# matteospanio/torchfx

Hardware: AMD Instinct MI355X
Metric: Msamples/s/GPU (64-ch fused biquad→FIR→FFT-conv chain); % HBM roofline (higher is better)
Workload: dtype f64 (IIR) + f32 (FFT); f32 I/O

## Files before the change

### torchfx_amd/csrc/ols_kernels.h

```cpp
#pragma once
#include "common.h"
#include "epilogue.h"
#include "fftpk.h"

namespace tfx {

typedef float2 cpx;

__device__ __forceinline__ cpx cmul(cpx a, cpx b) { return make_float2(a.x * b.x - a.y * b.y, a.x * b.y + a.y * b.x); }
__device__ __forceinline__ cpx cmulc(cpx a, cpx b) { return make_float2(a.x * b.x + a.y * b.y, a.y * b.x - a.x * b.y); }
__device__ __forceinline__ cpx cadd(cpx a, cpx b) { return make_float2(a.x + b.x, a.y + b.y); }
__device__ __forceinline__ cpx csub(cpx a, cpx b) { return make_float2(a.x - b.x, a.y - b.y); }

template <bool INV>
__device__ __forceinline__ void dft4(cpx &a0, cpx &a1, cpx &a2, cpx &a3)
{
    const cpx s02 = cadd(a0, a2), d02 = csub(a0, a2), s13 = cadd(a1, a3), d13 = csub(a1, a3);
    const cpx id = INV ? make_float2(-d13.y, d13.x) : make_float2(d13.y, -d13.x);
    a0 = cadd(s02, s13);
    a2 = csub(s02, s13);
    a1 = cadd(d02, id);
    a3 = csub(d02, id);
}

__device__ __forceinline__ void wave_sync2()
{
    __builtin_amdgcn_fence(__ATOMIC_RELEASE, "wavefront");
    __builtin_amdgcn_wave_barrier();
    __builtin_amdgcn_fence(__ATOMIC_ACQUIRE, "wavefront");
}

struct OlsGeom {
    int64_t Tn;
    int64_t Tout;
    int64_t F;
    int64_t S;
    int64_t t0;
    int64_t pad_left;
    int64_t out_shift;
    int64_t nframes;
    const float *hist;
    int64_t H;
    float ep_gain;
    int ep_scale, ep_clamp, ep_stat;
    double *ep_partial;
    int64_t ep_row;
    int N2;
    int P2;
    int sh_on, sh_base;
    int *nf_flag;
    int *nf_pair;
    int nt;
};

constexpr int OLS_N1 = 256;
constexpr int OLS_CB = 32;

__device__ __forceinline__ int pad16(int p) { return p + (p >> 4); }
__device__ __forceinline__ int row_shift(const OlsGeom &g, int64_t c) { return g.sh_on ? (int)(((int64_t)g.sh_base + c * g.Tn) & 31) : 0; }


template <bool INV, int NBF, bool LEAN = false>
__device__ __forceinline__ void col_stages16(cpx (&v)[NBF][16], cpx *lds, const cpx *tw256, int col, int q)
{
    constexpr int QS = 16 / NBF;
    using pk::v2f;
    const v2f Wc = {0.92387953251128675613f, 0.38268343236508977173f}, Wr = {0.70710678118654752440f, 0.70710678118654752440f};
    v2f *L = (v2f *)lds;
    const v2f *TW = (const v2f *)tw256;
#pragma unroll
    for (int i = 0; i < NBF; ++i) {
        v2f u[16];
#pragma unroll
        for (int t = 0; t < 16; ++t) u[t] = __builtin_bit_cast(v2f, v[i][t]);
        pk::pk_dft16<INV>(u, Wc, Wr);
        const int j = q + QS * i;
#pragma unroll
        for (int k = 0; k < 16; ++k) L[(16 * j + k) * OLS_CB + col] = u[PK_DFT16_AT(k)];
    }
    __syncthreads();
#pragma unroll
    for (int i = 0; i < NBF; ++i) {
        const int j = q + QS * i;
        v2f d[16], w[16];
#pragma unroll
        for (int t = 0; t < 16; ++t) d[t] = L[(j + 16 * t) * OLS_CB + col];
        if (LEAN) {
#pragma unroll
            for (int b = 0; b < 4; ++b) {
#pragma unroll
                for (int t = 0; t < 4; ++t) if (4 * b + t > 0) w[t] = TW[((4 * b + t) * j) & 255];
                __builtin_amdgcn_sched_barrier(0);
#pragma unroll
                for (int t = 0; t < 4; ++t) if (4 * b + t > 0) d[4 * b + t] = pk::pk_cmul<INV>(d[4 * b + t], w[t]);
            }
        } else {
#pragma unroll
            for (int t = 1; t < 16; ++t) w[t] = TW[(t * j) & 255];
            __builtin_amdgcn_sched_barrier(0);
#pragma unroll
            for (int t = 1; t < 16; ++t) d[t] = pk::pk_cmul<INV>(d[t], w[t]);
        }
        pk::pk_dft16<INV>(d, Wc, Wr);
#pragma unroll
        for (int t = 0; t < 16; ++t) v[i][t] = __builtin_bit_cast(cpx, d[t]);
    }
}

template <int NBF>
__global__ void __launch_bounds__(512 / NBF, 2)
ols_col_fwd16_kernel(const float *__restrict__ x, cpx *__restrict__ T, const cpx *__restrict__ tw256g,
                     OlsGeom g, int64_t frame0)
{
    constexpr int QS = 16 / NBF;
    extern __shared__ __attribute__((aligned(16))) char smem[];
    cpx *lds = (cpx *)smem;
    cpx *tw256 = lds + OLS_N1 * OLS_CB;
    const int tid = threadIdx.x, col = tid & 31, q = tid >> 5;
    if (tid < 256) tw256[tid] = tw256g[tid];
    const int ncb = g.N2 / OLS_CB;
    const int64_t pair = blockIdx.x / ncb;
    const int cb = blockIdx.x % ncb;
    const int n2 = cb * OLS_CB + col;
    const int64_t fa = frame0 + 2 * pair, fb = fa + 1;
    const int64_t ca = fa / g.F, ia0 = g.t0 + (fa % g.F) * g.S - g.pad_left - row_shift(g, ca);
    const bool has_b = fb < g.nframes;
    const int64_t cb_ = has_b ? fb / g.F : 0, ib0 = has_b ? g.t0 + (fb % g.F) * g.S - g.pad_left - row_shift(g, cb_) : 0;
    const float *xa = x + ca * g.Tn, *xb = x + cb_ * g.Tn;
    cpx v[NBF][16];
    const int64_t span = (int64_t)OLS_N1 * g.N2;
    const bool inner = ia0 >= 0 && ia0 + span <= g.Tn && has_b && ib0 >= 0 && ib0 + span <= g.Tn;
    if (inner && (g.nt & 1)) {
#pragma unroll
        for (int i = 0; i < NBF; ++i)
#pragma unroll
            for (int t = 0; t < 16; ++t) {
                const int64_t n = (int64_t)(q + QS * i + 16 * t) * g.N2 + n2;
                v[i][t] = make_float2(__builtin_nontemporal_load(xa + ia0 + n), __builtin_nontemporal_load(xb + ib0 + n));
            }
    } else if (inner) {
#pragma unroll
        for (int i = 0; i < NBF; ++i)
#pragma unroll
            for (int t = 0; t < 16; ++t) {
                const int64_t n = (int64_t)(q + QS * i + 16 * t) * g.N2 + n2;
                v[i][t] = make_float2(xa[ia0 + n], xb[ib0 + n]);
            }
    } else {
#pragma unroll
        for (int i = 0; i < NBF; ++i)
#pragma unroll
            for (int t = 0; t < 16; ++t) {
                const int64_t n = (int64_t)(q + QS * i + 16 * t) * g.N2 + n2;
                const int64_t ia = ia0 + n, ib = ib0 + n;
                float re = (ia >= 0 && ia < g.Tn) ? xa[ia] : 0.0f;
                float im = (has_b && ib >= 0 && ib < g.Tn) ? xb[ib] : 0.0f;
                if (g.hist) {
                    if (ia < 0 && ia >= -g.H) re = g.hist[ca * g.H + g.H + ia];
                    if (has_b && ib < 0 && ib >= -g.H) im = g.hist[cb_ * g.H + g.H + ib];
                }
                v[i][t] = make_float2(re, im);
            }
    }
    if (has_b && ca != cb_ && g.nf_pair) {
        bool bad = false;
#pragma unroll
        for (int i = 0; i < NBF; ++i)
#pragma unroll
            for (int t = 0; t < 16; ++t)
                if (!(__builtin_fabsf(v[i][t].y) <= 3.4028234663852886e38f)) { v[i][t].y = 0.0f; bad = true; }
        if (bad) g.nf_pair[cb_] = 1;
    }
    __syncthreads();
    col_stages16<false, NBF>(v, lds, tw256, col, q);
    cpx *Tp = T + pair * ((int64_t)OLS_N1 * g.P2);
#pragma unroll
    for (int i = 0; i < NBF; ++i)
#pragma unroll
        for (int k = 0; k < 16; ++k)
            Tp[(int64_t)(q + QS * i + 16 * k) * g.P2 + n2] = v[i][PK_DFT16_AT(k)];
}

template <int NBF>
__global__ void __launch_bounds__(512 / NBF, 2)
ols_col_inv16_kernel(const cpx *__restrict__ T, float *__restrict__ y, const cpx *__restrict__ tw256g,
                     OlsGeom g, int64_t frame0)
{
    constexpr int QS = 16 / NBF;
    extern __shared__ __attribute__((aligned(16))) char smem[];
    cpx *lds = (cpx *)smem;
    cpx *tw256 = lds + OLS_N1 * OLS_CB;
    const int tid = threadIdx.x, col = tid & 31, q = tid >> 5;
    if (tid < 256) tw256[tid] = tw256g[tid];
    const int ncb = g.N2 / OLS_CB;
    const int64_t pair = blockIdx.x / ncb;
    const int cb = blockIdx.x % ncb;
    const int n2 = cb * OLS_CB + col;
    const cpx *Tp = T + pair * ((int64_t)OLS_N1 * g.P2);
    cpx v[NBF][16];
#pragma unroll
    for (int i = 0; i < NBF; ++i)
#pragma unroll
        for (int t = 0; t < 16; ++t) v[i][t] = Tp[(int64_t)(q + QS * i + 16 * t) * g.P2 + n2];
    __syncthreads();
    col_stages16<true, NBF>(v, lds, tw256, col, q);

    const int64_t fa = frame0 + 2 * pair, fb = fa + 1;
    const int64_t ca = fa / g.F, oa0 = g.t0 + (fa % g.F) * g.S;
    const bool has_b = fb < g.nframes;
    const int64_t cb_ = has_b ? fb / g.F : 0, ob0 = has_b ? g.t0 + (fb % g.F) * g.S : 0;
    float *ya = y + ca * g.Tout, *yb = y + cb_ * g.Tout;
    const int64_t sha = g.out_shift + row_shift(g, ca), shb = g.out_shift + row_shift(g, cb_);
    const bool epi = g.ep_scale | g.ep_clamp | (g.ep_stat >= 0);
    double acc_a = 0.0, acc_b = 0.0;
#pragma unroll
    for (int i = 0; i < NBF; ++i)
#pragma unroll
        for (int k = 0; k < 16; ++k) {
            const int64_t n = (int64_t)(q + QS * i + 16 * k) * g.N2 + n2;
            if (n < g.S) {
                cpx o = v[i][PK_DFT16_AT(k)];
                const int64_t oa = oa0 + n - sha, ob = ob0 + n - shb;
                const bool wa = oa >= 0 && oa < g.Tout, wb = has_b && ob >= 0 && ob < g.Tout;
                if (epi) {
                    if (g.ep_scale) { o.x *= g.ep_gain; o.y *= g.ep_gain; }
                    if (g.ep_clamp) { o.x = clamp_unit(o.x); o.y = clamp_unit(o.y); }
                    if (g.ep_stat >= 0) {
                        if (wa) acc_a = red_comb_rt(g.ep_stat, acc_a, red_elem_rt(g.ep_stat, (double)o.x));
                        if (wb) acc_b = red_comb_rt(g.ep_stat, acc_b, red_elem_rt(g.ep_stat, (double)o.y));
                    }
                }
                if (g.nt & 2) {
                    if (wa) __builtin_nontemporal_store(o.x, ya + oa);
                    if (wb) __builtin_nontemporal_store(o.y, yb + ob);
                } else {
                    if (wa) ya[oa] = o.x;
                    if (wb) yb[ob] = o.y;
                }
            }
        }
    if (g.ep_stat >= 0) {
        double *red = (double *)smem;
        __syncthreads();
#pragma unroll
        for (int off = 32; off >= 1; off >>= 1) {
            acc_a = red_comb_rt(g.ep_stat, acc_a, __shfl_xor(acc_a, off));
            acc_b = red_comb_rt(g.ep_stat, acc_b, __shfl_xor(acc_b, off));
        }
        const int nw = (int)(blockDim.x >> 6), w = tid >> 6;
        if ((tid & 63) == 0) { red[w] = acc_a; red[nw + w] = acc_b; }
        __syncthreads();
        if (tid == 0) {
            double ra = red[0], rb = red[nw];
            for (int u = 1; u < nw; ++u) { ra = red_comb_rt(g.ep_stat, ra, red[u]); rb = red_comb_rt(g.ep_stat, rb, red[nw + u]); }
            g.ep_partial[ca * g.ep_row + (fa % g.F) * ncb + cb] = ra;
            if (has_b) g.ep_partial[cb_ * g.ep_row + (fb % g.F) * ncb + cb] = rb;
        }
    }
}

__global__ void __launch_bounds__(256) ols_straddle_fix_kernel(float *__restrict__ y, OlsGeom g)
{
    const int64_t c = blockIdx.x;
    if (!g.nf_pair[c]) return;
    if (blockIdx.y == 0 && threadIdx.x == 0 && g.ep_stat >= 0) g.ep_partial[c * g.ep_row] = __builtin_nan("");
    const int64_t lo = max((int64_t)0, g.t0 - g.out_shift - row_shift(g, c)), hi = min(g.Tout, g.t0 + g.S - g.out_shift - row_shift(g, c));
    for (int64_t t = lo + (int64_t)blockIdx.y * 256 + threadIdx.x; t < hi; t += (int64_t)gridDim.y * 256) y[c * g.Tout + t] = __builtin_nanf("");
}

constexpr int SOSF_MAXK = 8;
constexpr int SOSF_K4W = 4;
constexpr int SOSF_CH = 16;
constexpr int SOSF_LS = 36;
constexpr size_t OLS_SHM_SOSF = (size_t)512 * SOSF_LS * sizeof(float) + 256 * sizeof(cpx);
struct SosFuse {
    double co[SOSF_MAXK][5];
    double *sections;
    int warm_blocks;
    int prio;
};

template <int KS, bool TAPS, bool UNIT>
__global__ void __launch_bounds__(512, ((KS <= SOSF_K4W && !TAPS) ? 4 : 2))
ols_col_fwd16_sos_kernel(const float *__restrict__ x, cpx *__restrict__ T, const cpx *__restrict__ tw256g,
                         OlsGeom g, int64_t frame0, SosFuse sf)
{
    extern __shared__ __attribute__((aligned(16))) char smem[];
    float *S = (float *)smem;
    cpx *lds = (cpx *)smem;
    cpx *tw256 = (cpx *)(smem + (size_t)512 * SOSF_LS * sizeof(float));
    const int tid = threadIdx.x;
    if (tid < 256) tw256[tid] = tw256g[tid];
    const int64_t pair = blockIdx.x;
    const int64_t fa = frame0 + 2 * pair, fb = fa + 1;
    const int64_t ca = fa / g.F, ia0 = g.t0 + (fa % g.F) * g.S - g.pad_left - row_shift(g, ca);
    const bool has_b = fb < g.nframes;
    const int64_t cb_ = has_b ? fb / g.F : 0, ib0 = has_b ? g.t0 + (fb % g.F) * g.S - g.pad_left - row_shift(g, cb_) : 0;
    const float *xa = x + ca * g.Tn, *xb = x + cb_ * g.Tn;
    const int nblk = g.N2 / OLS_CB;
    int64_t ta = ia0 - (int64_t)OLS_CB * sf.warm_blocks, tb = ib0 - (int64_t)OLS_CB * sf.warm_blocks;
    auto bound = [](int64_t v) { return (int)(v < -(int64_t)0x40000000 ? -(int64_t)0x40000000 : (v > (int64_t)0x40000000 ? (int64_t)0x40000000 : v)); };

    const bool mine_b = tid >= 256;
    const int rel_l = (tid & 255) * g.N2;
    const int own_lo = TAPS ? ((((mine_b ? fb : fa) % g.F) == 0 && g.t0 == 0) ? 0 : OLS_N1 * g.N2 - (int)g.S) : 0;
    double h1[KS + 1], h2[KS + 1];
#pragma unroll
    for (int s = 0; s <= KS; ++s) { h1[s] = 0.0; h2[s] = 0.0; }

    const int lrow = tid >> 3, lpart = tid & 7;
    const int rel_f = lrow * g.N2 + 4 * lpart;
    const int rstep = 64 * g.N2;
    float4 P[8];
    auto fetch = [&]() {
        const float *pa = xa + ta, *pb = xb + tb;
        const int lo_a = bound(-ta), hi_a = bound(g.Tn - ta), lo_b = bound(-tb), hi_b = has_b ? bound(g.Tn - tb) : lo_b;
        int rel = rel_f;
        asm volatile("" : "+v"(rel));
#pragma unroll
        for (int i = 0; i < 8; ++i) {
            const bool isb = i >= 4;
            const int r = rel + (i & 3) * rstep;
            const int lo = isb ? lo_b : lo_a, hi = isb ? hi_b : hi_a;
            float4 v = make_float4(0.f, 0.f, 0.f, 0.f);
            if (r >= lo && r + 4 <= hi) {
                const float *src = (isb ? pb : pa) + r;
                v = (g.nt & 1) ? ldg16_stream<float4>(src) : *(const float4 *)src;
            } else if (r + 4 > lo && r < hi) {
                const float *src = (isb ? pb : pa) + r;
                if (r >= lo) v.x = src[0];
                if (r + 1 >= lo && r + 1 < hi) v.y = src[1];
                if (r + 2 >= lo && r + 2 < hi) v.z = src[2];
                if (r + 3 < hi) v.w = src[3];
            }
            P[i] = v;
        }
        ta += OLS_CB; tb += OLS_CB;
    };
    fetch();
    cpx *Tp = T + pair * ((int64_t)OLS_N1 * g.P2);
    const int col = tid & 31, q = tid >> 5;
    for (int blk = -sf.warm_blocks; blk < nblk; ++blk) {
#pragma unroll
        for (int i = 0; i < 8; ++i) *(float4 *)&S[(lrow + 64 * i) * SOSF_LS + 4 * lpart] = P[i];
        int64_t tcur = (mine_b ? tb : ta) - OLS_CB;
        {
            const unsigned lo32 = (unsigned)__builtin_amdgcn_readfirstlane((int)(unsigned)(uint64_t)tcur);
            const unsigned hi32 = (unsigned)__builtin_amdgcn_readfirstlane((int)(unsigned)((uint64_t)tcur >> 32));
            tcur = (int64_t)(((uint64_t)hi32 << 32) | lo32);
        }
        const int last = (!mine_b || has_b) ? min(max(bound(g.Tn - tcur) - rel_l, 0), OLS_CB) : 0;
        int first = 0;
        if (TAPS) first = max(min(max(bound(-tcur) - rel_l, 0), OLS_CB), min(max(own_lo - (rel_l + OLS_CB * blk), 0), OLS_CB));
        if (blk + 1 < nblk) fetch();
        __syncthreads();
        if (sf.prio) __builtin_amdgcn_s_setprio(0);
#pragma unroll 1
        for (int j = 0; j < OLS_CB / SOSF_CH; ++j) {
            float u[SOSF_CH];
#pragma unroll
            for (int i = 0; i < SOSF_CH / 4; ++i) {
                const float4 w4 = *(const float4 *)&S[tid * SOSF_LS + SOSF_CH * j + 4 * i];
                u[4 * i] = w4.x; u[4 * i + 1] = w4.y; u[4 * i + 2] = w4.z; u[4 * i + 3] = w4.w;
            }
            const int lastj = last - SOSF_CH * j, firstj = first - SOSF_CH * j;
#pragma unroll
            for (int n = 0; n < SOSF_CH; ++n) {
                double v = (double)u[n];
#pragma unroll
                for (int s = 0; s < KS; ++s) {
                    double yn = UNIT ? __builtin_fma(sf.co[s][1], h1[s], v) : __builtin_fma(sf.co[s][1], h1[s], sf.co[s][0] * v);
                    yn = __builtin_fma(sf.co[s][2], h2[s], yn);
                    yn = __builtin_fma(sf.co[s][3], h1[s + 1], yn);
                    yn = __builtin_fma(sf.co[s][4], h2[s + 1], yn);
                    h2[s] = h1[s]; h1[s] = v;
                    v = yn;
                    if (TAPS) {
                        if (blk >= 0 && n >= firstj && n < lastj)
                            sf.sections[((int64_t)s * (g.nframes / g.F) + (mine_b ? cb_ : ca)) * g.Tn + tcur + rel_l + SOSF_CH * j + n] =
                                UNIT ? yn * sf.co[s][0] : yn;
                    }
                }
                h2[KS] = h1[KS]; h1[KS] = v;
                if (UNIT) v *= sf.co[KS - 1][0];
                u[n] = n < lastj ? (float)v : 0.0f;
            }
            if (blk >= 0) {
#pragma unroll
                for (int i = 0; i < SOSF_CH / 4; ++i)
                    *(float4 *)&S[tid * SOSF_LS + SOSF_CH * j + 4 * i] = make_float4(u[4 * i], u[4 * i + 1], u[4 * i + 2], u[4 * i + 3]);
                if (!(__builtin_fabs(h1[KS]) <= 1.7976931348623157e308)) {
#pragma unroll
                    for (int i = 0; i < SOSF_CH / 4; ++i)
                        *(float4 *)&S[tid * SOSF_LS + SOSF_CH * j + 4 * i] = make_float4(0.f, 0.f, 0.f, 0.f);
                }
            }
        }
        if (sf.prio) __builtin_amdgcn_s_setprio(3);
        if (blk < 0) { __syncthreads(); continue; }
        __syncthreads();
        cpx v[1][16];
#pragma unroll
        for (int t = 0; t < 16; ++t) v[0][t] = make_float2(S[(q + 16 * t) * SOSF_LS + col], S[(256 + q + 16 * t) * SOSF_LS + col]);
        __syncthreads();
        col_stages16<false, 1, true>(v, lds, tw256, col, q);
        char *Tb = (char *)(Tp + blk * OLS_CB);
        unsigned off = (unsigned)(q * g.P2 + col) * (unsigned)sizeof(cpx);
        asm volatile("" : "+v"(off));
        const unsigned ostep = 16u * (unsigned)g.P2 * (unsigned)sizeof(cpx);
#pragma unroll
        for (int k = 0; k < 16; ++k) { *(cpx *)(Tb + off) = v[0][PK_DFT16_AT(k)]; off += ostep; }
        __syncthreads();
    }
    {
        int *flag = (int *)smem;
        if (tid < 2) flag[tid] = 0;
        __syncthreads();
        const double e1 = h1[KS], e2 = h2[KS];
        if (!(__builtin_fabs(e1) <= 1.7976931348623157e308 && __builtin_fabs(e2) <= 1.7976931348623157e308)) flag[mine_b ? 1 : 0] = 1;
        __syncthreads();
        if (tid == 0) g.nf_flag[fa] = flag[0];
        if (tid == 1 && has_b) g.nf_flag[fb] = flag[1];
    }
}

__global__ void __launch_bounds__(256)
ols_sos_nonfinite_fix_kernel(float *__restrict__ y, double *__restrict__ sections, OlsGeom g, int warm_blocks, OlsGeom gt, int has_tail)
{
    __shared__ int s_first;
    __shared__ long long s_n;
    const int tid = threadIdx.x;
    const int64_t c = blockIdx.x;
    if (tid == 0) { s_first = 0x7fffffff; s_n = 0x7fffffffffffffffll; }
    __syncthreads();
    for (int64_t f = tid; f < g.F; f += 256)
        if (g.nf_flag[c * g.F + f]) atomicMin(&s_first, (int)f);
    __syncthreads();
    int64_t first = s_first;
    if (first == 0x7fffffff) {
        if (!has_tail || !gt.nf_flag[c]) return;
        g = gt;
        first = 0;
    }
    const int sh = row_shift(g, c);
    const float nanf_ = __builtin_nanf("");
    if (blockIdx.z == 0) {
        if (blockIdx.y == 0 && tid == 0 && g.ep_stat >= 0) g.ep_partial[c * g.ep_row + first * (g.N2 / OLS_CB)] = __builtin_nan("");
        const int64_t t0 = max((int64_t)0, g.t0 + first * g.S - g.out_shift - sh);
        const int64_t len = g.Tout - t0, per = (len + gridDim.y - 1) / gridDim.y;
        const int64_t lo = t0 + per * blockIdx.y, hi = min(g.Tout, lo + per);
        for (int64_t t = lo + tid; t < hi; t += 256) y[c * g.Tout + t] = nanf_;
        return;
    }
    if (!sections || blockIdx.y != 0) return;
    double *row = sections + ((int64_t)(blockIdx.z - 1) * (g.nframes / g.F) + c) * g.Tn;
    const int64_t start = max((int64_t)0, g.t0 + first * g.S - g.pad_left - sh - (int64_t)OLS_CB * warm_blocks);
    for (int64_t t0 = start; t0 < g.Tn; t0 += 4096) {
        for (int64_t t = t0 + tid; t < min(g.Tn, t0 + 4096); t += 256)
            if (!(__builtin_fabs(row[t]) <= 1.7976931348623157e308)) { atomicMin(&s_n, (long long)t); break; }
        __syncthreads();
        if (s_n != 0x7fffffffffffffffll) break;
    }
    const int64_t n = s_n;
    if (n == 0x7fffffffffffffffll) return;
    const double nan_ = __builtin_nan("");
    for (int64_t t = n + 1 + tid; t < g.Tn; t += 256) row[t] = nan_;
}

template <int L2, bool INV>
__device__ __forceinline__ void row_stages(cpx (&v)[(1 << (2 * L2)) / 256][4], cpx *lds, const cpx *twr, int lane)
{
    constexpr int N2 = 1 << (2 * L2), Q = N2 / 4, NB = Q / 64;
#pragma unroll
    for (int i = 0; i < NB; ++i) dft4<INV>(v[i][0], v[i][1], v[i][2], v[i][3]);
#pragma unroll
    for (int s = 1; s < L2; ++s) {
        const int Ns_prev = 1 << (2 * (s - 1));
        const int Ns = Ns_prev * 4;
#pragma unroll
        for (int i = 0; i < NB; ++i) {
            const int j = lane + 64 * i;
            const int j0 = (j / Ns_prev) * (4 * Ns_prev) + (j % Ns_prev);
#pragma unroll
            for (int r = 0; r < 4; ++r) lds[j0 + r * Ns_prev] = v[i][r];
        }
        wave_sync2();
#pragma unroll
        for (int i = 0; i < NB; ++i) {
            const int j = lane + 64 * i;
            const int k = j % Ns;
#pragma unroll
            for (int r = 0; r < 4; ++r) {
                cpx x = lds[j + Q * r];
                if (r > 0) {
                    const cpx w = twr[(r * k * (Q / Ns)) & (N2 - 1)];
                    x = INV ? cmulc(x, w) : cmul(x, w);
                }
                v[i][r] = x;
            }
            dft4<INV>(v[i][0], v[i][1], v[i][2], v[i][3]);
        }
        wave_sync2();
    }
}

template <int L2>
__global__ void __launch_bounds__(256)
ols_row_kernel(cpx *__restrict__ T, const cpx *__restrict__ Hp, const cpx *__restrict__ twrg,
               const cpx *__restrict__ tlo, const cpx *__restrict__ thi, int64_t nrows, int P2)
{
    constexpr int N2 = 1 << (2 * L2), Q = N2 / 4, NB = Q / 64;
    constexpr int64_t N = (int64_t)OLS_N1 * N2;
    extern __shared__ __attribute__((aligned(16))) char smem[];
    cpx *twr = (cpx *)smem;
    const int tid = threadIdx.x, lane = tid & 63, wave = tid >> 6;
    cpx *lds = twr + N2 + wave * N2;
    for (int i = tid; i < N2; i += 256) twr[i] = twrg[i];
    __syncthreads();
    const int64_t row = (int64_t)blockIdx.x * 4 + wave;
    if (row >= nrows) return;
    const int k1 = (int)(row % OLS_N1);
    cpx *base = T + row * P2;
    const cpx *hrow = Hp + (int64_t)k1 * N2;

    cpx v[NB][4], w[NB][4];
#pragma unroll
    for (int i = 0; i < NB; ++i) {
#pragma unroll
        for (int r = 0; r < 4; ++r) {
            const int n2 = lane + 64 * i + Q * r;
            const unsigned m = (unsigned)(((int64_t)k1 * n2) & (N - 1));
            w[i][r] = cmul(tlo[m & 511], thi[m >> 9]);
            v[i][r] = cmul(base[n2], w[i][r]);
        }
    }
    row_stages<L2, false>(v, lds, twr, lane);
#pragma unroll
    for (int i = 0; i < NB; ++i)
#pragma unroll
        for (int r = 0; r < 4; ++r) v[i][r] = cmul(v[i][r], hrow[lane + 64 * i + Q * r]);
    row_stages<L2, true>(v, lds, twr, lane);
#pragma unroll
    for (int i = 0; i < NB; ++i)
#pragma unroll
        for (int r = 0; r < 4; ++r) base[lane + 64 * i + Q * r] = cmulc(v[i][r], w[i][r]);
}

__global__ void __launch_bounds__(256, 3)
ols_row256pk_kernel(cpx *__restrict__ T, const cpx *__restrict__ Hp, const cpx *__restrict__ tw256g,
                    const cpx *__restrict__ tlo, const cpx *__restrict__ thi, int64_t nrows, int P2)
{
    using pk::v2f;
    extern __shared__ __attribute__((aligned(16))) char smem[];
    const int tid = threadIdx.x, lane = tid & 63, wave = tid >> 6, i = lane & 15, r = lane >> 4;
    v2f *L = (v2f *)smem + (wave * 4 + r) * 272;
    const v2f Wc = {0.92387953251128675613f, 0.38268343236508977173f}, Wr = {0.70710678118654752440f, 0.70710678118654752440f};
    v2f tw[16];
#pragma unroll
    for (int k = 1; k < 16; ++k) tw[k] = ((const v2f *)tw256g)[(i * k) & 255];
    for (int64_t row0 = ((int64_t)blockIdx.x * 4 + wave) * 4; row0 < nrows; row0 += (int64_t)gridDim.x * 16) {
        const int64_t row = row0 + r;
        const bool live = row < nrows;
        const int k1 = (int)((live ? row : 0) % OLS_N1);
        v2f *base = (v2f *)(T + (live ? row : 0) * P2);
        const v2f *hrow = (const v2f *)(Hp + (int64_t)k1 * 256);
        v2f w[16];
        {
            const unsigned ma = (unsigned)(k1 * i), mb = (unsigned)(16 * k1);
            const v2f wl = pk::pk_cmul<false>(((const v2f *)tlo)[ma & 511], ((const v2f *)thi)[ma >> 9]);
            v2f u[16];
            u[1] = pk::pk_cmul<false>(((const v2f *)tlo)[mb & 511], ((const v2f *)thi)[mb >> 9]);
            u[2] = pk::pk_cmul<false>(u[1], u[1]);
            u[3] = pk::pk_cmul<false>(u[2], u[1]);
            u[4] = pk::pk_cmul<false>(u[2], u[2]);
            u[5] = pk::pk_cmul<false>(u[4], u[1]);
            u[6] = pk::pk_cmul<false>(u[4], u[2]);
            u[7] = pk::pk_cmul<false>(u[4], u[3]);
            u[8] = pk::pk_cmul<false>(u[4], u[4]);
#pragma unroll
            for (int t = 9; t < 16; ++t) u[t] = pk::pk_cmul<false>(u[8], u[t - 8]);
            w[0] = wl;
#pragma unroll
            for (int t = 1; t < 16; ++t) w[t] = pk::pk_cmul<false>(wl, u[t]);
        }
        v2f v[16];
#pragma unroll
        for (int t = 0; t < 16; ++t) v[t] = live ? base[i + 16 * t] : v2f{0.f, 0.f};
        __builtin_amdgcn_sched_barrier(0);
#pragma unroll
        for (int t = 0; t < 16; ++t) v[t] = pk::pk_cmul<false>(v[t], w[t]);
        pk::pk_dft16<false>(v, Wc, Wr);
        L[17 * i] = v[PK_DFT16_AT(0)];
#pragma unroll
        for (int k = 1; k < 16; ++k) L[17 * i + k] = pk::pk_cmul<false>(v[PK_DFT16_AT(k)], tw[k]);
        wave_sync2();
#pragma unroll
        for (int t = 0; t < 16; ++t) v[t] = L[17 * t + i];
        wave_sync2();
        pk::pk_dft16<false>(v, Wc, Wr);
        v2f h[16];
#pragma unroll
        for (int k = 0; k < 16; ++k) h[k] = hrow[i + 16 * k];
        __builtin_amdgcn_sched_barrier(0);
        v2f z[16];
#pragma unroll
        for (int k = 0; k < 16; ++k) z[k] = pk::pk_cmul<false>(v[PK_DFT16_AT(k)], h[k]);
        pk::pk_dft16<true>(z, Wc, Wr);
        L[17 * i] = z[PK_DFT16_AT(0)];
#pragma unroll
        for (int k = 1; k < 16; ++k) L[17 * i + k] = pk::pk_cmul<true>(z[PK_DFT16_AT(k)], tw[k]);
        wave_sync2();
#pragma unroll
        for (int t = 0; t < 16; ++t) z[t] = L[17 * t + i];
        wave_sync2();
        pk::pk_dft16<true>(z, Wc, Wr);
        if (live) {
#pragma unroll
            for (int t = 0; t < 16; ++t) base[i + 16 * t] = pk::pk_cmul<true>(z[PK_DFT16_AT(t)], w[t]);
        }
    }
}

template <bool INV>
__device__ __forceinline__ void row_fft1024_pk(pk::v2f (&v)[16], pk::v2f *lds, const pk::v2f *twr, int lane, pk::v2f Wc, pk::v2f Wr)
{
    using pk::v2f;
    pk::pk_dft16<INV>(v, Wc, Wr);
#pragma unroll
    for (int k = 0; k < 16; ++k) lds[pad16(16 * lane + k)] = v[PK_DFT16_AT(k)];
    wave_sync2();
    const int kb = lane & 15;
    {
        v2f d[16], w[16];
#pragma unroll
        for (int t = 0; t < 16; ++t) d[t] = lds[pad16(lane + 64 * t)];
#pragma unroll
        for (int t = 1; t < 16; ++t) w[t] = twr[(4 * t * kb) & 1023];
        __builtin_amdgcn_sched_barrier(0);
        v[0] = d[0];
#pragma unroll
        for (int t = 1; t < 16; ++t) v[t] = pk::pk_cmul<INV>(d[t], w[t]);
    }
    wave_sync2();
    pk::pk_dft16<INV>(v, Wc, Wr);
    const int j0 = (lane >> 4) * 256 + kb;
#pragma unroll
    for (int k = 0; k < 16; ++k) lds[pad16(j0 + 16 * k)] = v[PK_DFT16_AT(k)];
    wave_sync2();
    {
        v2f d[16], w[16];
#pragma unroll
        for (int i = 0; i < 4; ++i)
#pragma unroll
            for (int r = 0; r < 4; ++r) {
                d[i + 4 * r] = lds[pad16(lane + 64 * i + 256 * r)];
                if (r > 0) w[i + 4 * r] = twr[(r * (lane + 64 * i)) & 1023];
            }
        __builtin_amdgcn_sched_barrier(0);
#pragma unroll
        for (int i = 0; i < 4; ++i) {
#pragma unroll
            for (int r = 1; r < 4; ++r) d[i + 4 * r] = pk::pk_cmul<INV>(d[i + 4 * r], w[i + 4 * r]);
            pk::pk_dft4<INV, false>(d[i], d[i + 4], d[i + 8], d[i + 12]);
        }
#pragma unroll
        for (int t = 0; t < 16; ++t) v[t] = d[t];
    }
    wave_sync2();
}

__global__ void __launch_bounds__(256, 3)
ols_row1024_kernel(cpx *__restrict__ T, const cpx *__restrict__ Hp, const cpx *__restrict__ twrg,
                   const cpx *__restrict__ tlo, const cpx *__restrict__ thi, const cpx *__restrict__ tu,
                   int64_t nrows, int64_t Nmask, int P2)
{
    constexpr int N2 = 1024, LDSROW = N2 + N2 / 16;
    extern __shared__ __attribute__((aligned(16))) char smem[];
    cpx *twr = (cpx *)smem;
    const int tid = threadIdx.x, lane = tid & 63;
    const int wave = __builtin_amdgcn_readfirstlane(tid >> 6);
    cpx *lds = twr + N2 + wave * LDSROW;
    for (int i = tid; i < N2; i += 256) twr[i] = twrg[i];
    __syncthreads();
    const int64_t row = (int64_t)blockIdx.x * 4 + wave;
    if (row >= nrows) return;
    const int k1 = (int)(row % OLS_N1);
    cpx *base = T + row * P2;
    const cpx *hrow = Hp + (int64_t)k1 * N2;
    typedef const float __attribute__((address_space(4))) *cfp;
    const cfp tuc = (cfp)(uintptr_t)tu;

    const unsigned ml = (unsigned)(k1 * lane);
    const cpx wl = cmul(tlo[ml & 511], thi[ml >> 9]);
    using pk::v2f;
    const v2f Wc = {0.92387953251128675613f, 0.38268343236508977173f}, Wr = {0.70710678118654752440f, 0.70710678118654752440f};
    v2f u[16], h[16];
#pragma unroll
    for (int t = 0; t < 16; ++t) h[t] = ((const v2f *)base)[lane + 64 * t];
    __builtin_amdgcn_sched_barrier(0);
#pragma unroll
    for (int t = 0; t < 16; ++t) {
        const unsigned iu = 2u * ((unsigned)(k1 * t) & (unsigned)(Nmask >> 6));
        const cpx w = cmul(wl, make_float2(tuc[iu], tuc[iu + 1]));
        u[t] = pk::pk_cmul<false>(h[t], __builtin_bit_cast(v2f, w));
    }
    row_fft1024_pk<false>(u, (v2f *)lds, (const v2f *)twr, lane, Wc, Wr);
    __builtin_amdgcn_sched_barrier(0);
#pragma unroll
    for (int t = 0; t < 16; ++t) h[t] = ((const v2f *)hrow)[lane + 64 * t];
    __builtin_amdgcn_sched_barrier(0);
#pragma unroll
    for (int t = 0; t < 16; ++t) u[t] = pk::pk_cmul<false>(u[t], h[t]);
    __builtin_amdgcn_sched_barrier(0);
    row_fft1024_pk<true>(u, (v2f *)lds, (const v2f *)twr, lane, Wc, Wr);
    float wlx = wl.x, wly = wl.y;
    asm volatile("" : "+v"(wlx), "+v"(wly));
    const cpx wl2 = make_float2(wlx, wly);
#pragma unroll
    for (int t = 0; t < 16; ++t) {
        const unsigned iu = 2u * ((unsigned)(k1 * t) & (unsigned)(Nmask >> 6));
        const cpx w = cmul(wl2, make_float2(tuc[iu], tuc[iu + 1]));
        ((v2f *)base)[lane + 64 * t] = pk::pk_cmul<true>(u[t], __builtin_bit_cast(v2f, w));
    }
}

template <int MAP>
__global__ void __launch_bounds__(256, 4)
ols_row4096_kernel(cpx *__restrict__ T, const cpx *__restrict__ Hp, const cpx *__restrict__ tw256g,
                   const cpx *__restrict__ t4log, const cpx *__restrict__ t4hig,
                   const cpx *__restrict__ tlo, const cpx *__restrict__ thi, const cpx *__restrict__ tu,
                   int64_t Nmask, int P2, int64_t npairs)
{
    constexpr int N2 = 4096;
    extern __shared__ __attribute__((aligned(16))) char smem[];
    cpx *lds = (cpx *)smem;
    cpx *twB = lds + N2 + N2 / 16;
    cpx *twA = twB + 256;
    const int j = threadIdx.x;
    twB[j] = tw256g[((j >> 4) * (j & 15)) & 255];
    twA[j] = t4log[j];
    typedef const float __attribute__((address_space(4))) *cfp;
    const cfp tuc = (cfp)(uintptr_t)tu;
    const unsigned umask = (unsigned)(Nmask >> 8);
    int k1;
    int64_t p;
    if (MAP == 0) {
        k1 = (int)(blockIdx.x % OLS_N1);
        p = blockIdx.x / OLS_N1;
    } else {
        const unsigned xcd = blockIdx.x & 7u, m = blockIdx.x >> 3;
        k1 = (int)((m / (unsigned)npairs) * 8u + xcd);
        p = m % (unsigned)npairs;
    }
    __syncthreads();
    const cpx *hrow = Hp + (int64_t)k1 * N2;
    const unsigned ml = (unsigned)(k1 * j);
    const cpx wl = cmul(tlo[ml & 511], thi[ml >> 9]);
    cpx *base = T + (p * OLS_N1 + k1) * P2;
    using pk::v2f;
    const v2f Wc = {0.92387953251128675613f, 0.38268343236508977173f}, Wr = {0.70710678118654752440f, 0.70710678118654752440f};
    v2f u[16], h[16];
#pragma unroll
    for (int t = 0; t < 16; ++t) h[t] = ((const v2f *)base)[j + 256 * t];
    __builtin_amdgcn_sched_barrier(0);
#pragma unroll
    for (int t = 0; t < 16; ++t) {
        const unsigned iu = 2u * ((unsigned)(k1 * t) & umask);
        const cpx w = cmul(wl, make_float2(tuc[iu], tuc[iu + 1]));
        u[t] = pk::pk_cmul<false>(h[t], __builtin_bit_cast(v2f, w));
    }
    pk::fft4096_pk<false>(u, (v2f *)lds, (const v2f *)twB, (const v2f *)twA, j, Wc, Wr);
    __builtin_amdgcn_sched_barrier(0);
#pragma unroll
    for (int t = 0; t < 16; ++t) h[t] = ((const v2f *)hrow)[j + 256 * t];
    __builtin_amdgcn_sched_barrier(0);
#pragma unroll
    for (int t = 0; t < 16; ++t) u[t] = pk::pk_cmul<false>(u[t], h[t]);
    __builtin_amdgcn_sched_barrier(0);
    pk::fft4096_pk<true>(u, (v2f *)lds, (const v2f *)twB, (const v2f *)twA, j, Wc, Wr);
    float wlx = wl.x, wly = wl.y;
    asm volatile("" : "+v"(wlx), "+v"(wly));
    const cpx wl2 = make_float2(wlx, wly);
#pragma unroll
    for (int t = 0; t < 16; ++t) {
        const unsigned iu = 2u * ((unsigned)(k1 * t) & umask);
        const cpx w = cmul(wl2, make_float2(tuc[iu], tuc[iu + 1]));
        ((v2f *)base)[j + 256 * t] = pk::pk_cmul<true>(u[t], __builtin_bit_cast(v2f, w));
    }
}


__device__ __forceinline__ int row8192_at(int k2)
{
    const int h = k2 & 1, m = k2 >> 1, t = m >> 8, jj = m & 255;
    return ((h * 8 + (t >> 1)) * 256 + jj) * 2 + (t & 1);
}
inline int row8192_at_host(int k2)
{
    const int h = k2 & 1, m = k2 >> 1, t = m >> 8, jj = m & 255;
    return ((h * 8 + (t >> 1)) * 256 + jj) * 2 + (t & 1);
}

template <int MAP>
__global__ void __launch_bounds__(256, 4)
ols_row8192_kernel(cpx *__restrict__ T, const cpx *__restrict__ Hp, const cpx *__restrict__ tw256g,
                   const cpx *__restrict__ t4log, const cpx *__restrict__ tlo, const cpx *__restrict__ thi,
                   const cpx *__restrict__ tu, const cpx *__restrict__ w8kg, int64_t Nmask, int P2, int64_t npairs)
{
    using pk::v2f;
    using pk::v4f;
    constexpr int N2 = 8192;
    extern __shared__ __attribute__((aligned(16))) char smem[];
    cpx *lds = (cpx *)smem;
    cpx *twBc = lds + 4096 + 256;
    cpx *twAc = twBc + 256;
    const int j = threadIdx.x;
    twBc[j] = tw256g[((j >> 4) * (j & 15)) & 255];
    twAc[j] = t4log[j];
    typedef const float __attribute__((address_space(4))) *cfp;
    const cfp tuc = (cfp)(uintptr_t)tu;
    const unsigned umask = (unsigned)(Nmask >> 8);
    int k1;
    int64_t p;
    if (MAP == 0) {
        k1 = (int)(blockIdx.x % OLS_N1);
        p = blockIdx.x / OLS_N1;
    } else {
        const unsigned xcd = blockIdx.x & 7u, m = blockIdx.x >> 3;
        k1 = (int)((m / (unsigned)npairs) * 8u + xcd);
        p = m % (unsigned)npairs;
    }
    const v2f wj = ((const v2f *)w8kg)[j];
    __syncthreads();
    const v2f *twB = (const v2f *)twBc, *twA = (const v2f *)twAc;
    const v4f *Hq = (const v4f *)(Hp + (int64_t)k1 * N2);
    const unsigned ml = (unsigned)(k1 * j);
    const cpx wl = cmul(tlo[ml & 511], thi[ml >> 9]);
    cpx *base = T + (p * OLS_N1 + k1) * P2;
    const v2f Wc = {0.92387953251128675613f, 0.38268343236508977173f}, Wr = {0.70710678118654752440f, 0.70710678118654752440f};
    char *rowb = (char *)base;
    unsigned roff = (unsigned)j * (unsigned)sizeof(cpx);
    asm volatile("" : "+v"(roff));
    v2f a[16], b[16];
#pragma unroll
    for (int half = 0; half < 2; ++half) {
        v2f lo[8], hi[8];
#pragma unroll
        for (int u = 0; u < 8; ++u) {
            const int t = 8 * half + u;
            lo[u] = *(const v2f *)(rowb + (roff + 2048u * (unsigned)t));
            hi[u] = *(const v2f *)(rowb + (roff + 2048u * (unsigned)(t + 16)));
        }
        __builtin_amdgcn_sched_barrier(0);
#pragma unroll
        for (int u = 0; u < 8; ++u) {
            const int t = 8 * half + u;
            const unsigned i0 = 2u * ((unsigned)(k1 * t) & umask), i1 = 2u * ((unsigned)(k1 * (t + 16)) & umask);
            const cpx w0 = cmul(wl, make_float2(tuc[i0], tuc[i0 + 1])), w1 = cmul(wl, make_float2(tuc[i1], tuc[i1 + 1]));
            const v2f l = pk::pk_cmul<false>(lo[u], __builtin_bit_cast(v2f, w0)), h = pk::pk_cmul<false>(hi[u], __builtin_bit_cast(v2f, w1));
            const v2f w = t ? pk::pk_cmul<false>(wj, twB[16 * t + 8]) : wj;
            a[t] = l + h;
            b[t] = pk::pk_cmul<false>(l - h, w);
        }
        __builtin_amdgcn_sched_barrier(0);
    }
    pk::fft4096_pk<false>(a, (v2f *)lds, twB, twA, j, Wc, Wr);
    {
        v4f q[8];
#pragma unroll
        for (int m = 0; m < 8; ++m) q[m] = Hq[m * 256 + j];
        __builtin_amdgcn_sched_barrier(0);
#pragma unroll
        for (int m = 0; m < 8; ++m) {
            a[2 * m] = pk::pk_cmul<false>(a[2 * m], v2f{q[m].x, q[m].y});
            a[2 * m + 1] = pk::pk_cmul<false>(a[2 * m + 1], v2f{q[m].z, q[m].w});
        }
    }
    pk::fft4096_pk<false>(b, (v2f *)lds, twB, twA, j, Wc, Wr);
    {
        v4f q[8];
#pragma unroll
        for (int m = 0; m < 8; ++m) q[m] = Hq[(8 + m) * 256 + j];
        __builtin_amdgcn_sched_barrier(0);
#pragma unroll
        for (int m = 0; m < 8; ++m) {
            b[2 * m] = pk::pk_cmul<false>(b[2 * m], v2f{q[m].x, q[m].y});
            b[2 * m + 1] = pk::pk_cmul<false>(b[2 * m + 1], v2f{q[m].z, q[m].w});
        }
    }
    pk::fft4096_pk<true>(a, (v2f *)lds, twB, twA, j, Wc, Wr);
    pk::fft4096_pk<true>(b, (v2f *)lds, twB, twA, j, Wc, Wr);
    float wlx = wl.x, wly = wl.y;
    asm volatile("" : "+v"(wlx), "+v"(wly));
    const cpx wl2 = make_float2(wlx, wly);
    v2f wj2 = wj;
    asm volatile("" : "+v"(wj2));
    unsigned roff2 = (unsigned)j * (unsigned)sizeof(cpx);
    asm volatile("" : "+v"(roff2));
#pragma unroll
    for (int t = 0; t < 16; ++t) {
        const v2f w = t ? pk::pk_cmul<false>(wj2, twB[16 * t + 8]) : wj2;
        const v2f bw = pk::pk_cmul<true>(b[t], w);
        const unsigned i0 = 2u * ((unsigned)(k1 * t) & umask), i1 = 2u * ((unsigned)(k1 * (t + 16)) & umask);
        const cpx w0 = cmul(wl2, make_float2(tuc[i0], tuc[i0 + 1])), w1 = cmul(wl2, make_float2(tuc[i1], tuc[i1 + 1]));
        *(v2f *)(rowb + (roff2 + 2048u * (unsigned)t)) = pk::pk_cmul<true>(a[t] + bw, __builtin_bit_cast(v2f, w0));
        *(v2f *)(rowb + (roff2 + 2048u * (unsigned)(t + 16))) = pk::pk_cmul<true>(a[t] - bw, __builtin_bit_cast(v2f, w1));
    }
}

__global__ void __launch_bounds__(256, 4)
ols_rowspec4096_kernel(cpx *__restrict__ T, const cpx *__restrict__ tw256g, const cpx *__restrict__ t4log,
                       const cpx *__restrict__ tlo, const cpx *__restrict__ thi, const cpx *__restrict__ tu,
                       int64_t Nmask, int P2, float inv_n)
{
    using pk::v2f;
    extern __shared__ __attribute__((aligned(16))) char smem[];
    cpx *lds = (cpx *)smem;
    cpx *twB = lds + 4096 + 256;
    cpx *twA = twB + 256;
    const int j = threadIdx.x;
    twB[j] = tw256g[((j >> 4) * (j & 15)) & 255];
    twA[j] = t4log[j];
    typedef const float __attribute__((address_space(4))) *cfp;
    const cfp tuc = (cfp)(uintptr_t)tu;
    const unsigned umask = (unsigned)(Nmask >> 8);
    const int k1 = (int)blockIdx.x;
    __syncthreads();
    const unsigned ml = (unsigned)(k1 * j);
    const cpx wl = cmul(tlo[ml & 511], thi[ml >> 9]);
    cpx *base = T + (int64_t)k1 * P2;
    const v2f Wc = {0.92387953251128675613f, 0.38268343236508977173f}, Wr = {0.70710678118654752440f, 0.70710678118654752440f};
    v2f u[16];
#pragma unroll
    for (int t = 0; t < 16; ++t) {
        const unsigned iu = 2u * ((unsigned)(k1 * t) & umask);
        const cpx w = cmul(wl, make_float2(tuc[iu], tuc[iu + 1]));
        u[t] = pk::pk_cmul<false>(((const v2f *)base)[j + 256 * t], __builtin_bit_cast(v2f, w));
    }
    pk::fft4096_pk<false>(u, (v2f *)lds, (const v2f *)twB, (const v2f *)twA, j, Wc, Wr);
#pragma unroll
    for (int t = 0; t < 16; ++t) base[j + 256 * t] = make_float2(u[t].x * inv_n, -u[t].y * inv_n);
}

__global__ void __launch_bounds__(256, 4)
ols_rowspec8192_kernel(cpx *__restrict__ T, const cpx *__restrict__ tw256g, const cpx *__restrict__ t4log,
                       const cpx *__restrict__ tlo, const cpx *__restrict__ thi, const cpx *__restrict__ tu,
                       const cpx *__restrict__ w8kg, int64_t Nmask, int P2, float inv_n)
{
    using pk::v2f;
    extern __shared__ __attribute__((aligned(16))) char smem[];
    cpx *lds = (cpx *)smem;
    cpx *twBc = lds + 4096 + 256;
    cpx *twAc = twBc + 256;
    const int j = threadIdx.x;
    twBc[j] = tw256g[((j >> 4) * (j & 15)) & 255];
    twAc[j] = t4log[j];
    typedef const float __attribute__((address_space(4))) *cfp;
    const cfp tuc = (cfp)(uintptr_t)tu;
    const unsigned umask = (unsigned)(Nmask >> 8);
    const int k1 = (int)blockIdx.x;
    const v2f wj = ((const v2f *)w8kg)[j];
    __syncthreads();
    const v2f *twB = (const v2f *)twBc, *twA = (const v2f *)twAc;
    const unsigned ml = (unsigned)(k1 * j);
    const cpx wl = cmul(tlo[ml & 511], thi[ml >> 9]);
    cpx *base = T + (int64_t)k1 * P2;
    const v2f Wc = {0.92387953251128675613f, 0.38268343236508977173f}, Wr = {0.70710678118654752440f, 0.70710678118654752440f};
    v2f a[16], b[16];
#pragma unroll
    for (int t = 0; t < 16; ++t) {
        const unsigned i0 = 2u * ((unsigned)(k1 * t) & umask), i1 = 2u * ((unsigned)(k1 * (t + 16)) & umask);
        const cpx w0 = cmul(wl, make_float2(tuc[i0], tuc[i0 + 1])), w1 = cmul(wl, make_float2(tuc[i1], tuc[i1 + 1]));
        const v2f l = pk::pk_cmul<false>(((const v2f *)base)[j + 256 * t], __builtin_bit_cast(v2f, w0));
        const v2f h = pk::pk_cmul<false>(((const v2f *)base)[j + 256 * (t + 16)], __builtin_bit_cast(v2f, w1));
        const v2f w = t ? pk::pk_cmul<false>(wj, twB[16 * t + 8]) : wj;
        a[t] = l + h;
        b[t] = pk::pk_cmul<false>(l - h, w);
    }
    pk::fft4096_pk<false>(a, (v2f *)lds, twB, twA, j, Wc, Wr);
    pk::fft4096_pk<false>(b, (v2f *)lds, twB, twA, j, Wc, Wr);
#pragma unroll
    for (int t = 0; t < 16; ++t) {
        base[((0 * 8 + (t >> 1)) * 256 + j) * 2 + (t & 1)] = make_float2(a[t].x * inv_n, -a[t].y * inv_n);
        base[((1 * 8 + (t >> 1)) * 256 + j) * 2 + (t & 1)] = make_float2(b[t].x * inv_n, -b[t].y * inv_n);
    }
}

}
```

Measured before the change: 193,500.

## Restructure SOS-fused column FFT kernel with per-wave loads and fewer block barriers

Each wave now fetches input rows only for its own frame (a or b), so the load-to-LDS staging is wave-local and the post-staging block barrier becomes a lighter wave_sync2. The first column FFT stage now runs in place on the float staging buffer S instead of being copied into a separate complex LDS array, which removes a gather pass and one barrier. The trailing barrier at the end of each block is removed, and warm-up blocks sync only at the wave level except on the last one. This cuts LDS traffic and block-wide synchronisation, at the cost of depending on subtle cross-wave ordering, since S is reused between iterations without a closing barrier.

```diff
diff --git a/torchfx_amd/csrc/ols_kernels.h b/torchfx_amd/csrc/ols_kernels.h
--- a/torchfx_amd/csrc/ols_kernels.h
+++ b/torchfx_amd/csrc/ols_kernels.h
@@ -60,7 +60,7 @@
 __device__ __forceinline__ int row_shift(const OlsGeom &g, int64_t c) { return g.sh_on ? (int)(((int64_t)g.sh_base + c * g.Tn) & 31) : 0; }
 
 
-template <bool INV, int NBF, bool LEAN = false>
+template <bool INV, int NBF>
 __device__ __forceinline__ void col_stages16(cpx (&v)[NBF][16], cpx *lds, const cpx *tw256, int col, int q)
 {
     constexpr int QS = 16 / NBF;
@@ -85,22 +85,11 @@
         v2f d[16], w[16];
 #pragma unroll
         for (int t = 0; t < 16; ++t) d[t] = L[(j + 16 * t) * OLS_CB + col];
-        if (LEAN) {
-#pragma unroll
-            for (int b = 0; b < 4; ++b) {
-#pragma unroll
-                for (int t = 0; t < 4; ++t) if (4 * b + t > 0) w[t] = TW[((4 * b + t) * j) & 255];
-                __builtin_amdgcn_sched_barrier(0);
-#pragma unroll
-                for (int t = 0; t < 4; ++t) if (4 * b + t > 0) d[4 * b + t] = pk::pk_cmul<INV>(d[4 * b + t], w[t]);
-            }
-        } else {
-#pragma unroll
-            for (int t = 1; t < 16; ++t) w[t] = TW[(t * j) & 255];
-            __builtin_amdgcn_sched_barrier(0);
-#pragma unroll
-            for (int t = 1; t < 16; ++t) d[t] = pk::pk_cmul<INV>(d[t], w[t]);
-        }
+#pragma unroll
+        for (int t = 1; t < 16; ++t) w[t] = TW[(t * j) & 255];
+        __builtin_amdgcn_sched_barrier(0);
+#pragma unroll
+        for (int t = 1; t < 16; ++t) d[t] = pk::pk_cmul<INV>(d[t], w[t]);
         pk::pk_dft16<INV>(d, Wc, Wr);
 #pragma unroll
         for (int t = 0; t < 16; ++t) v[i][t] = __builtin_bit_cast(cpx, d[t]);
@@ -280,6 +269,37 @@
     int prio;
 };
 
+__device__ __forceinline__ void col_stages16_stage(cpx (&v)[1][16], float *S, const cpx *tw256, int col, int q)
+{
+    using pk::v2f;
+    const v2f Wc = {0.92387953251128675613f, 0.38268343236508977173f}, Wr = {0.70710678118654752440f, 0.70710678118654752440f};
+    const v2f *TW = (const v2f *)tw256;
+    asm volatile("" : "+v"(q));
+    float *Sa = S + q * SOSF_LS + col, *Sb = Sa + 256 * SOSF_LS;
+    v2f d[16], w[4];
+#pragma unroll
+    for (int t = 0; t < 16; ++t) d[t] = v2f{Sa[16 * t * SOSF_LS], Sb[16 * t * SOSF_LS]};
+    pk::pk_dft16<false>(d, Wc, Wr);
+#pragma unroll
+    for (int k = 0; k < 16; ++k) { const v2f o = d[PK_DFT16_AT(k)]; Sa[16 * k * SOSF_LS] = o.x; Sb[16 * k * SOSF_LS] = o.y; }
+    __syncthreads();
+    const float *Ra = S + 16 * q * SOSF_LS + col, *Rb = Ra + 256 * SOSF_LS;
+#pragma unroll
+    for (int t = 0; t < 16; ++t) d[t] = v2f{Ra[t * SOSF_LS], Rb[t * SOSF_LS]};
+    __syncthreads();
+#pragma unroll
+    for (int b = 0; b < 4; ++b) {
+#pragma unroll
+        for (int t = 0; t < 4; ++t) if (4 * b + t > 0) w[t] = TW[((4 * b + t) * q) & 255];
+        __builtin_amdgcn_sched_barrier(0);
+#pragma unroll
+        for (int t = 0; t < 4; ++t) if (4 * b + t > 0) d[4 * b + t] = pk::pk_cmul<false>(d[4 * b + t], w[t]);
+    }
+    pk::pk_dft16<false>(d, Wc, Wr);
+#pragma unroll
+    for (int t = 0; t < 16; ++t) v[0][t] = __builtin_bit_cast(cpx, d[t]);
+}
+
 template <int KS, bool TAPS, bool UNIT>
 __global__ void __launch_bounds__(512, ((KS <= SOSF_K4W && !TAPS) ? 4 : 2))
 ols_col_fwd16_sos_kernel(const float *__restrict__ x, cpx *__restrict__ T, const cpx *__restrict__ tw256g,
@@ -287,7 +307,6 @@
 {
     extern __shared__ __attribute__((aligned(16))) char smem[];
     float *S = (float *)smem;
-    cpx *lds = (cpx *)smem;
     cpx *tw256 = (cpx *)(smem + (size_t)512 * SOSF_LS * sizeof(float));
     const int tid = threadIdx.x;
     if (tid < 256) tw256[tid] = tw256g[tid];
@@ -298,36 +317,36 @@
     const int64_t cb_ = has_b ? fb / g.F : 0, ib0 = has_b ? g.t0 + (fb % g.F) * g.S - g.pad_left - row_shift(g, cb_) : 0;
     const float *xa = x + ca * g.Tn, *xb = x + cb_ * g.Tn;
     const int nblk = g.N2 / OLS_CB;
-    int64_t ta = ia0 - (int64_t)OLS_CB * sf.warm_blocks, tb = ib0 - (int64_t)OLS_CB * sf.warm_blocks;
+    const bool mine_b = __builtin_amdgcn_readfirstlane(tid >> 8) != 0;
+    int64_t tw = (mine_b ? ib0 : ia0) - (int64_t)OLS_CB * sf.warm_blocks;
+    const float *xw = mine_b ? xb : xa;
+    const bool has_w = !mine_b || has_b;
     auto bound = [](int64_t v) { return (int)(v < -(int64_t)0x40000000 ? -(int64_t)0x40000000 : (v > (int64_t)0x40000000 ? (int64_t)0x40000000 : v)); };
 
-    const bool mine_b = tid >= 256;
     const int rel_l = (tid & 255) * g.N2;
     const int own_lo = TAPS ? ((((mine_b ? fb : fa) % g.F) == 0 && g.t0 == 0) ? 0 : OLS_N1 * g.N2 - (int)g.S) : 0;
     double h1[KS + 1], h2[KS + 1];
 #pragma unroll
     for (int s = 0; s <= KS; ++s) { h1[s] = 0.0; h2[s] = 0.0; }
 
-    const int lrow = tid >> 3, lpart = tid & 7;
-    const int rel_f = lrow * g.N2 + 4 * lpart;
-    const int rstep = 64 * g.N2;
+    const int lline = (tid & ~63) + ((tid & 63) >> 3), lpart = tid & 7;
+    const int rel_f = (lline & 255) * g.N2 + 4 * lpart;
+    const int rstep = 8 * g.N2;
     float4 P[8];
     auto fetch = [&]() {
-        const float *pa = xa + ta, *pb = xb + tb;
-        const int lo_a = bound(-ta), hi_a = bound(g.Tn - ta), lo_b = bound(-tb), hi_b = has_b ? bound(g.Tn - tb) : lo_b;
+        const float *pw = xw + tw;
+        const int lo = bound(-tw), hi = has_w ? bound(g.Tn - tw) : lo;
         int rel = rel_f;
         asm volatile("" : "+v"(rel));
 #pragma unroll
         for (int i = 0; i < 8; ++i) {
-            const bool isb = i >= 4;
-            const int r = rel + (i & 3) * rstep;
-            const int lo = isb ? lo_b : lo_a, hi = isb ? hi_b : hi_a;
+            const int r = rel + i * rstep;
             float4 v = make_float4(0.f, 0.f, 0.f, 0.f);
             if (r >= lo && r + 4 <= hi) {
-                const float *src = (isb ? pb : pa) + r;
+                const float *src = pw + r;
                 v = (g.nt & 1) ? ldg16_stream<float4>(src) : *(const float4 *)src;
             } else if (r + 4 > lo && r < hi) {
-                const float *src = (isb ? pb : pa) + r;
+                const float *src = pw + r;
                 if (r >= lo) v.x = src[0];
                 if (r + 1 >= lo && r + 1 < hi) v.y = src[1];
                 if (r + 2 >= lo && r + 2 < hi) v.z = src[2];
@@ -335,25 +354,20 @@
             }
             P[i] = v;
         }
-        ta += OLS_CB; tb += OLS_CB;
+        tw += OLS_CB;
     };
     fetch();
     cpx *Tp = T + pair * ((int64_t)OLS_N1 * g.P2);
     const int col = tid & 31, q = tid >> 5;
     for (int blk = -sf.warm_blocks; blk < nblk; ++blk) {
 #pragma unroll
-        for (int i = 0; i < 8; ++i) *(float4 *)&S[(lrow + 64 * i) * SOSF_LS + 4 * lpart] = P[i];
-        int64_t tcur = (mine_b ? tb : ta) - OLS_CB;
-        {
-            const unsigned lo32 = (unsigned)__builtin_amdgcn_readfirstlane((int)(unsigned)(uint64_t)tcur);
-            const unsigned hi32 = (unsigned)__builtin_amdgcn_readfirstlane((int)(unsigned)((uint64_t)tcur >> 32));
-            tcur = (int64_t)(((uint64_t)hi32 << 32) | lo32);
-        }
+        for (int i = 0; i < 8; ++i) *(float4 *)&S[(lline + 8 * i) * SOSF_LS + 4 * lpart] = P[i];
+        const int64_t tcur = tw - OLS_CB;
         const int last = (!mine_b || has_b) ? min(max(bound(g.Tn - tcur) - rel_l, 0), OLS_CB) : 0;
         int first = 0;
         if (TAPS) first = max(min(max(bound(-tcur) - rel_l, 0), OLS_CB), min(max(own_lo - (rel_l + OLS_CB * blk), 0), OLS_CB));
         if (blk + 1 < nblk) fetch();
-        __syncthreads();
+        wave_sync2();
         if (sf.prio) __builtin_amdgcn_s_setprio(0);
 #pragma unroll 1
         for (int j = 0; j < OLS_CB / SOSF_CH; ++j) {
@@ -397,20 +411,20 @@
             }
         }
         if (sf.prio) __builtin_amdgcn_s_setprio(3);
-        if (blk < 0) { __syncthreads(); continue; }
+        if (blk < 0) {
+            wave_sync2();
+            if (blk == -1) __syncthreads();
+            continue;
+        }
         __syncthreads();
         cpx v[1][16];
-#pragma unroll
-        for (int t = 0; t < 16; ++t) v[0][t] = make_float2(S[(q + 16 * t) * SOSF_LS + col], S[(256 + q + 16 * t) * SOSF_LS + col]);
-        __syncthreads();
-        col_stages16<false, 1, true>(v, lds, tw256, col, q);
+        col_stages16_stage(v, S, tw256, col, q);
         char *Tb = (char *)(Tp + blk * OLS_CB);
         unsigned off = (unsigned)(q * g.P2 + col) * (unsigned)sizeof(cpx);
         asm volatile("" : "+v"(off));
         const unsigned ostep = 16u * (unsigned)g.P2 * (unsigned)sizeof(cpx);
 #pragma unroll
         for (int k = 0; k < 16; ++k) { *(cpx *)(Tb + off) = v[0][PK_DFT16_AT(k)]; off += ostep; }
-        __syncthreads();
     }
     {
         int *flag = (int *)smem;
```

Measured after the change: 194,100 (median of 5 runs). Within noise of the previous version (+0.3%).
